# ratschlab/secedo

Hardware: AMD Instinct MI355X
Metric: cell-pair x locus updates/sec (similarity matrix) (higher is better)
Workload: dtype int64

## Files before the change

### secedo_amd/csrc/pack_device.hip

```cpp
#include "pack_device.hpp"

#include <hip/hip_runtime.h>
#include <hipcub/hipcub.hpp>

#include <algorithm>
#include <chrono>
#include <cstdio>
#include <cstdlib>
#include <cstring>

namespace secedo {

DeviceArena::~DeviceArena() {
    if (p) (void)hipFree(p);
}

DevicePacked::~DevicePacked() {
    if (side) (void)hipStreamDestroy(side);
    if (ev_fork) (void)hipEventDestroy(ev_fork);
    if (ev_join) (void)hipEventDestroy(ev_join);
    if (ev_offsets) (void)hipEventDestroy(ev_offsets);
    if (ev_flush) (void)hipEventDestroy(ev_flush);
    if (mailbox) (void)hipHostFree(mailbox);
}
// ... 861 lines not shown
            if (split[t] != cut) {
                split[t] = cut;
                sc->split_changed = 1;
            }
            l_prev = l_t;
        }
    }
}

__device__ __forceinline__ unsigned long long bin_key(uint32_t blk, uint32_t l, uint32_t cib, uint32_t lbits) {
    return ((((unsigned long long)blk << lbits) | l) << kCibBits) | cib;
}

__global__ void k_keys2(Raw in, const uint32_t *sval, const unsigned long long *incl,
                        const uint32_t *read_locus, const uint32_t *run_rank, const uint32_t *read_off,
                        uint32_t num_cells, uint32_t B,
                        uint32_t lbits, unsigned long long *key2, uint32_t *val2, uint32_t *t_read,
                        uint32_t *krank, uint8_t *kflags, unsigned long long *entry_kc, const uint32_t *entry_map,
                        uint32_t *blk_cnt_add, uint32_t L, Scalars *sc) {
    const uint32_t n = in.n_entries;
    for (uint32_t s = blockIdx.x * TPB + threadIdx.x; s < n; s += gridDim.x * TPB) {
        const unsigned long long cur = incl[s], prev = s ? incl[s - 1] : 0ull;
        const uint32_t e_out = entry_map ? entry_map[sval[s]] : sval[s];
        if (incl_kept(cur) == incl_kept(prev)) {
            if (entry_kc) entry_kc[e_out] = kNoEntry;
            continue;
        }
        const uint32_t k = incl_kept(prev);
        const uint32_t group = in.id_base(sval[s]) >> 2;
        uint32_t cell = 0;
        if (group >= in.n_groups) {
            sc->error = 1;
        } else {
            cell = in.g2p[group];
            if (cell >= num_cells) {
                sc->error = 2;
                cell = 0;
            }
        }
        const uint32_t blk = cell / B, cib = cell - blk * B;
        if (key2) {
            key2[k] = bin_key(blk, read_locus[k], cib, lbits);
            val2[k] = k;
        }
        const uint32_t r = incl_reads(cur) - 1;
        t_read[k] = r;
        krank[k] = run_rank[r];
        kflags[k] = (uint8_t)((in.id_base(sval[s]) & 3u) | (read_off[r + 1] - read_off[r] > 1u ? 4u : 0u));
        if (entry_kc) entry_kc[e_out] = ((unsigned long long)((blk << kCibBits) | cib) << 32) | k;
        if (blk_cnt_add) atomicAdd(&blk_cnt_add[(size_t)blk * (L + 1) + read_locus[k]], 1u);
    }
}

__device__ __forceinline__ uint32_t tile_locus(const uint32_t *s_off, uint32_t lo, uint32_t hi, uint32_t e) {
    while (hi - lo > 1u) {
        const uint32_t mid = (lo + hi) >> 1;
        if (s_off[mid] <= e) lo = mid; else hi = mid;
    }
    return lo;
}

__global__ __launch_bounds__(TPB) void k_bin_hist(Raw in, uint32_t nb, uint32_t TL, unsigned long long *__restrict__ entry_kc,
                                                 const uint32_t *__restrict__ m_idx, uint32_t num_cells,
                                                 uint32_t B_log2, uint32_t *__restrict__ blk_cnt, Scalars *sc,
                                                 uint32_t g2p_lds) {
    extern __shared__ uint32_t lds_hist[];
    __shared__ uint32_t s_off[65];
    static_assert(TPB >= 65, "one thread per offset");
    const uint32_t L = in.n_loci, TLP = TL + 1u, TL_log2 = 31u - (uint32_t)__clz((int)TL);
    const uint32_t n_tiles = (L + TL - 1u) / TL;
    constexpr int U = 4;
    uint16_t *s_g2p = reinterpret_cast<uint16_t *>(lds_hist + nb * TLP);
    if (g2p_lds) {
        for (uint32_t i = threadIdx.x; i < in.n_groups; i += TPB) s_g2p[i] = (uint16_t)min(in.g2p[i], 0xFFFFu);
    }
    for (uint32_t tile = blockIdx.x; tile < n_tiles; tile += gridDim.x) {
        const uint32_t l0 = tile * TL, n_l = min(TL, L - l0);
        for (uint32_t i = threadIdx.x; i < nb * TLP; i += TPB) lds_hist[i] = 0;
        if (threadIdx.x <= n_l) s_off[threadIdx.x] = (uint32_t)in.locus_entry_off[l0 + threadIdx.x];
        __syncthreads();
        const uint32_t eb = s_off[0], ee = s_off[n_l];
        for (uint32_t base = eb + threadIdx.x; base < ee; base += TPB * U) {
            uint32_t slot[U];
            constexpr uint32_t kNone = 0xFFFFFFFFu;
            if (m_idx) {
                uint32_t m0[U], m1[U], ib[U], cell[U];
#pragma unroll
                for (int u = 0; u < U; ++u) {
                    const uint32_t e = base + (uint32_t)u * TPB;
                    const bool in_tile = e < ee;
                    m0[u] = in_tile ? m_idx[e] : 0u;
                    m1[u] = in_tile ? m_idx[e + 1] : 1u;
                    ib[u] = in_tile ? in.id_base(e) : 0u;
                }
#pragma unroll
                for (int u = 0; u < U; ++u) {
                    const uint32_t group = ib[u] >> 2;
                    cell[u] = 0;
                    if (m1[u] == m0[u]) {
                        if (group >= in.n_groups) sc->error = 1;
                        else cell[u] = g2p_lds ? (uint32_t)s_g2p[group] : in.g2p[group];
                    }
                }
#pragma unroll
                for (int u = 0; u < U; ++u) {
                    slot[u] = kNone;
                    if (m1[u] != m0[u]) continue;
                    const uint32_t e = base + (uint32_t)u * TPB;
                    uint32_t c = cell[u];
                    if (c >= num_cells) {
                        sc->error = 2;
                        c = 0;
                    }
                    const uint32_t blk = c >> B_log2, cib = c - (blk << B_log2);
                    entry_kc[e] = ((unsigned long long)(((ib[u] & 3u) << kSingleBaseShift) | (blk << kCibBits) | cib) << 32)
                            | kSingle;
                    slot[u] = blk;
                }
            } else {
#pragma unroll
                for (int u = 0; u < U; ++u) {
                    const uint32_t e = base + (uint32_t)u * TPB;
                    const unsigned long long kc = e < ee ? entry_kc[e] : (unsigned long long)kNoEntry;
                    slot[u] = (uint32_t)kc != kNoEntry ? (uint32_t)(kc >> 32) >> kCibBits : kNone;
                }
            }
#pragma unroll
            for (int u = 0; u < U; ++u) {
                if (slot[u] == kNone) continue;
                const uint32_t j = tile_locus(s_off, 0u, n_l, base + (uint32_t)u * TPB);
                atomicAdd(&lds_hist[slot[u] * TLP + j], 1u);
            }
        }
        __syncthreads();
        for (uint32_t i = threadIdx.x; i < nb * TL; i += TPB) {
            const uint32_t b = i >> TL_log2, j = i & (TL - 1u);
            if (j < n_l) {
                blk_cnt[(size_t)b * (L + 1) + l0 + j] = lds_hist[b * TLP + j];
                if (l0 + j == L - 1) blk_cnt[(size_t)b * (L + 1) + L] = 0;
            }
        }
        __syncthreads();
    }
}

__global__ __launch_bounds__(TPB) void k_bin_place(Raw in, uint32_t nb, uint32_t TL,
                                                  const unsigned long long *__restrict__ entry_kc,
                                                  const uint32_t *__restrict__ blk_off, uint32_t B_log2, uint32_t bm_words,
                                                  const uint32_t *tail_begin,
                                                  unsigned long long *__restrict__ grouped, uint8_t *dupflag) {
    extern __shared__ uint32_t lds_hist[];
    __shared__ uint32_t s_off[65];
    __shared__ uint32_t s_tail[64];
    constexpr uint32_t NW = TPB / 64;
    constexpr int D = 4;
    const uint32_t lane = threadIdx.x & 63u, wv = threadIdx.x >> 6, L = in.n_loci, TLP = TL + 1u;
    const uint32_t TL_log2 = 31u - (uint32_t)__clz((int)TL);
    uint32_t *bm = lds_hist + nb * TLP + wv * bm_words;
    for (uint32_t i = lane; i < bm_words; i += 64u) bm[i] = 0;
    const uint32_t n_tiles = (L + TL - 1u) / TL;
    for (uint32_t tile = blockIdx.x; tile < n_tiles; tile += gridDim.x) {
        const uint32_t l0 = tile * TL, n_l = min(TL, L - l0);
        for (uint32_t i = threadIdx.x; i < nb * TL; i += TPB) {
            const uint32_t b = i >> TL_log2, j = i & (TL - 1u);
            if (j < n_l) lds_hist[b * TLP + j] = blk_off[(size_t)b * (L + 1) + l0 + j];
        }
        if (threadIdx.x <= n_l) s_off[threadIdx.x] = (uint32_t)in.locus_entry_off[l0 + threadIdx.x];
        if (threadIdx.x < n_l)
            s_tail[threadIdx.x] = tail_begin
                    ? tail_begin[last_le<uint32_t>(in.chr_locus_off, in.n_chr + 1, l0 + threadIdx.x)] : 0u;
        __syncthreads();
        const uint32_t per_wave = (n_l + NW - 1u) / NW;
        const uint32_t ja = min(n_l, wv * per_wave), jb = min(n_l, ja + per_wave);
        const uint32_t E0 = s_off[ja], E1 = s_off[jb];
        uint32_t cur = ja;
        bool twice = bm_words == 0u;
        auto close_locus = [&]() {
            const bool any_twice = __ballot(twice) != 0ull;
            if (lane == 0u) dupflag[l0 + cur] = any_twice ? 1 : 0;
            if (bm_words) {
                __builtin_amdgcn_fence(__ATOMIC_RELEASE, "wavefront");
                __builtin_amdgcn_wave_barrier();
                for (uint32_t i = lane; i < bm_words; i += 64u) bm[i] = 0;
                __builtin_amdgcn_fence(__ATOMIC_RELEASE, "wavefront");
                __builtin_amdgcn_wave_barrier();
            }
            twice = bm_words == 0u;
            ++cur;
        };
        auto chunk = [&](unsigned long long kc, uint32_t base) {
            const uint32_t e = base + lane;
            const bool valid = e < E1;
            const uint32_t j = valid ? tile_locus(s_off, cur, jb, e) : 0xFFFFFFFFu;
            const uint32_t chunk_end = min(E1, base + 64u);
            while (true) {
                if (valid && j == cur) {
                    uint32_t k = (uint32_t)kc;
                    if (k != kNoEntry) {
                        uint32_t cc = (uint32_t)(kc >> 32);
                        if (k & kSingle) {
                            k = kSingle | (e >= s_tail[cur] ? kSingleTail : 0u) | (cc >> kSingleBaseShift);
                            cc &= (1u << kSingleBaseShift) - 1u;
                        }
                        if (bm_words) {
                            const uint32_t cell = ((cc >> kCibBits) << B_log2) + (cc & ((1u << kCibBits) - 1u));
                            const uint32_t bit = 1u << (cell & 31u);
                            twice |= (atomicOr(&bm[cell >> 5], bit) & bit) != 0u;
                        }
                        const uint32_t pos = atomicAdd(&lds_hist[(cc >> kCibBits) * TLP + cur], 1u);
                        grouped[pos] = ((unsigned long long)((cc & ((1u << kCibBits) - 1u)) | ((l0 + cur) << kCibBits)) << 32) | k;
                    }
                }
                if (s_off[cur + 1] > chunk_end) break;
                close_locus();
                if (cur >= jb) break;
            }
        };
        unsigned long long ring[D];
#pragma unroll
        for (int d = 0; d < D; ++d) {
            const uint32_t e = E0 + (uint32_t)d * 64u + lane;
            ring[d] = e < E1 ? entry_kc[e] : (unsigned long long)kNoEntry;
        }
        for (uint32_t base = E0; base < E1; base += 64u * D) {
#pragma unroll
            for (int d = 0; d < D; ++d) {
                const uint32_t b = base + (uint32_t)d * 64u;
                if (b >= E1) break;
                const unsigned long long kc = ring[d];
                const uint32_t nxt = b + 64u * D + lane;
                ring[d] = nxt < E1 ? entry_kc[nxt] : (unsigned long long)kNoEntry;
                chunk(kc, b);
            }
        }
        while (cur < jb) close_locus();
        __syncthreads();
    }
}

__global__ __launch_bounds__(TPB) void k_group_counts(const unsigned long long *skey2, uint32_t n, uint32_t B,
                                                     uint32_t L, uint32_t lbits, uint32_t *blk_cnt,
                                                     unsigned long long *per_cell_sq) {
    constexpr uint32_t SLOTS = 512;
    __shared__ unsigned long long sq[SLOTS];
    __shared__ uint32_t first_cell;
    const uint32_t per_block = (n + gridDim.x - 1) / gridDim.x;
    const uint32_t d0 = blockIdx.x * per_block, d1 = min(n, d0 + per_block);
    for (uint32_t i = threadIdx.x; i < SLOTS; i += TPB) sq[i] = 0;
    if (threadIdx.x == 0 && d0 < n) {
        const unsigned long long key = skey2[d0];
        first_cell = (uint32_t)(key >> (kCibBits + lbits)) * B;
    }
    __syncthreads();
    for (uint32_t d = d0 + threadIdx.x; d < d1; d += TPB) {
        const unsigned long long key = skey2[d];
        const unsigned long long grp = key >> kCibBits;
        const uint32_t blk = (uint32_t)(grp >> lbits), l = (uint32_t)grp & ((1u << lbits) - 1u);
        if (d == 0 || skey2[d - 1] >> kCibBits != grp) {
            uint32_t len = 1;
            for (uint32_t t = d + 1; t < n && skey2[t] >> kCibBits == grp; ++t) ++len;
            blk_cnt[(size_t)blk * (L + 1) + l] = len;
        }
        if (d == 0 || skey2[d - 1] != key) {
            unsigned long long cnt = 1;
            for (uint32_t t = d + 1; t < n && skey2[t] == key; ++t) ++cnt;
            const uint32_t cell = blk * B + ((uint32_t)key & ((1u << kCibBits) - 1u));
            const uint32_t rel = cell - first_cell;
            if (rel < SLOTS) atomicAdd(&sq[rel], cnt * cnt);
            else atomicAdd(&per_cell_sq[cell], cnt * cnt);
        }
    }
    __syncthreads();
    if (d0 < n) {
        for (uint32_t i = threadIdx.x; i < SLOTS; i += TPB) {
            if (sq[i]) atomicAdd(&per_cell_sq[first_cell + i], sq[i]);
        }
    }
}

struct CapChoice {
    uint32_t entries_plain, loci_plain;
    uint32_t entries_counts, loci_counts;
    unsigned long long count_limit;
    uint32_t allow_counts;
    __device__ __forceinline__ bool counts(const Scalars *sc) const {
        return allow_counts && sc->pair_bound < count_limit;
    }
};

__global__ __launch_bounds__(TPB) void k_ranges_segment(const uint32_t *blk_off, uint32_t nb, uint32_t L,
// ... 124 lines not shown
        const uint32_t k = sval2[d];
        const uint32_t cib = (uint32_t)key & ((1u << kCibBits) - 1u);
        const unsigned long long grp = key >> kCibBits;
        const uint32_t blk = (uint32_t)(grp >> lbits), l = (uint32_t)grp & ((1u << lbits) - 1u);
        const uint32_t cell = blk * B + cib;
        const uint32_t fl = kflags[k];
        const uint32_t base = fl & 3u;
        const bool multi = (fl & 4u) != 0u;
        const uint32_t chr = locus_chr[l];
        const bool tail = krank[k] - rbeg[chr] >= flushed[chr];
        uint32_t r = 0, lo = k, hi = k + 1;
        if (multi) {
            r = t_read[k];
            lo = read_off[r];
            hi = read_off[r + 1];
        }
        uint32_t meta = cell | (base << kMetaBaseShift) | (tail ? kMetaTail : 0u);
        uint32_t masks = 0, bases = 0;
        bool wide = false;
        for (uint32_t j = k; j-- > lo;) {
            const uint32_t dist = l - read_locus[j];
            if (dist > kNarrowWindow) wide = true;
            if (dist > kWindow) {
                meta |= kMetaPrevOvf;
                break;
            }
            masks |= 1u << (dist - 1);
        }
        for (uint32_t j = k + 1; j < hi; ++j) {
            const uint32_t dist = read_locus[j] - l;
            if (dist > kNarrowWindow) wide = true;
            if (dist > kWindow) {
                meta |= kMetaNextOvf;
                break;
            }
            masks |= 1u << (16 + dist - 1);
            bases |= (uint32_t)(read_base[j] & 1u) << (dist - 1);
            bases |= (uint32_t)((read_base[j] >> 1) & 1u) << (16 + dist - 1);
        }
        if (multi || tail) {
            entry[d] = make_uint4(meta, masks, bases, l);
            entry_read[d] = r;
        }
        entry32[d] = cib | (base << kC_BaseShift) | (tail ? kC_Tail : 0u) | (multi ? kC_Multi : 0u)
                | (wide ? kC_Wide : 0u) | ((locus_rel[l] & 0xFFFFu) << 16);
        if (mask32)
            mask32[d] = (masks & 0xFFu) | (((masks >> 16) & 0xFFu) << 8) | ((bases & 0xFFu) << 16)
                    | (((bases >> 16) & 0xFFu) << 24);
        n_wide += wide ? 1u : 0u;
    }
    if (n_wide) atomicAdd(&sc->n_wide, n_wide);
}

constexpr uint32_t kRecMulti = 1u << 30, kRecWide = 1u << 31;
__global__ void k_m_records(Raw in, uint32_t n_kept_m, const uint32_t *t_read, const uint32_t *read_off,
                            const uint32_t *read_locus, const uint8_t *read_base, const uint32_t *krank,
                            const uint8_t *kflags, const uint32_t *rbeg, const uint32_t *flushed, uint4 *m_rec,
                            Scalars *sc) {
    __shared__ uint32_t s_chr[1025];
    const bool chr_lds = in.n_chr <= 1024u;
    if (chr_lds)
        for (uint32_t i = threadIdx.x; i <= in.n_chr; i += TPB) s_chr[i] = in.chr_locus_off[i];
    __syncthreads();
    uint32_t n_wide = 0;
    for (uint32_t k = blockIdx.x * TPB + threadIdx.x; k < n_kept_m; k += gridDim.x * TPB) {
        const uint32_t fl = kflags[k], l = read_locus[k];
        const bool multi = (fl & 4u) != 0u;
        const uint32_t chr = chr_lds ? last_le<uint32_t>(s_chr, in.n_chr + 1, l)
                                     : last_le<uint32_t>(in.chr_locus_off, in.n_chr + 1, l);
        const bool tail = krank[k] - rbeg[chr] >= flushed[chr];
        uint32_t r = 0, lo = k, hi = k + 1;
        if (multi) {
            r = t_read[k];
            lo = read_off[r];
            hi = read_off[r + 1];
        }
        uint32_t meta = ((fl & 3u) << kMetaBaseShift) | (tail ? kMetaTail : 0u) | (multi ? kRecMulti : 0u);
        uint32_t masks = 0, bases = 0;
        for (uint32_t j = k; j-- > lo;) {
            const uint32_t dist = l - read_locus[j];
            if (dist > kNarrowWindow) meta |= kRecWide;
            if (dist > kWindow) {
                meta |= kMetaPrevOvf;
                break;
            }
            masks |= 1u << (dist - 1);
        }
        for (uint32_t j = k + 1; j < hi; ++j) {
            const uint32_t dist = read_locus[j] - l;
            if (dist > kNarrowWindow) meta |= kRecWide;
            if (dist > kWindow) {
                meta |= kMetaNextOvf;
                break;
            }
            masks |= 1u << (16 + dist - 1);
            bases |= (uint32_t)(read_base[j] & 1u) << (dist - 1);
            bases |= (uint32_t)((read_base[j] >> 1) & 1u) << (16 + dist - 1);
        }
        m_rec[k] = make_uint4(meta, masks, bases, r);
        n_wide += (meta & kRecWide) ? 1u : 0u;
    }
    if (n_wide) atomicAdd(&sc->n_wide, n_wide);
}

struct RecordTables {
    const uint4 *m_rec;
    const uint32_t *locus_rel;
    uint4 *entry;
    uint32_t *entry32, *mask32, *entry_read;
};

__device__ __forceinline__ void emit_record(const RecordTables &t, uint32_t d, uint32_t k, uint4 rec, uint32_t cib,
                                            uint32_t cell, uint32_t l, uint32_t lrel) {
    uint32_t base, meta, masks = 0, bases = 0, r = 0;
    bool multi = false, wide = false, tail;
    if (k & kSingle) {
        base = k & 3u;
        tail = (k & kSingleTail) != 0u;
        meta = cell | (base << kMetaBaseShift) | (tail ? kMetaTail : 0u);
    } else {
        base = (rec.x >> kMetaBaseShift) & 3u;
        tail = (rec.x & kMetaTail) != 0u;
        multi = (rec.x & kRecMulti) != 0u;
        wide = (rec.x & kRecWide) != 0u;
        meta = cell | (rec.x & ~(kRecMulti | kRecWide));
        masks = rec.y;
        bases = rec.z;
        r = rec.w;
    }
    if (multi || tail) {
        t.entry[d] = make_uint4(meta, masks, bases, l);
        t.entry_read[d] = r;
    }
    t.entry32[d] = cib | (base << kC_BaseShift) | (tail ? kC_Tail : 0u) | (multi ? kC_Multi : 0u)
            | (wide ? kC_Wide : 0u) | (lrel << 16);
    if (t.mask32)
        t.mask32[d] = (masks & 0xFFu) | (((masks >> 16) & 0xFFu) << 8) | ((bases & 0xFFu) << 16)
                | (((bases >> 16) & 0xFFu) << 24);
}

constexpr int TPB_REC = 512;
__global__ __launch_bounds__(TPB_REC) void k_entry_records(const unsigned long long *grouped, const uint32_t *blk_off,
                                                          uint32_t n, uint32_t nb, uint32_t L, uint32_t B,
                                                          uint32_t lbits, RecordTables t,
                                                          unsigned long long *per_cell_sq, Scalars *sc) {
    constexpr uint32_t SLOTS = 512;
    __shared__ unsigned long long sq[SLOTS];
    __shared__ uint32_t blk_start[1025];
    __shared__ uint32_t first_cell;
    const uint32_t per_block = (n + gridDim.x - 1) / gridDim.x;
    const uint32_t d0 = blockIdx.x * per_block, d1 = min(n, d0 + per_block);
    for (uint32_t i = threadIdx.x; i < SLOTS; i += TPB_REC) sq[i] = 0;
    for (uint32_t i = threadIdx.x; i <= nb; i += TPB_REC) blk_start[i] = i < nb ? blk_off[(size_t)i * (L + 1)] : n;
    __syncthreads();
    auto block_of = [&](uint32_t p) {
        uint32_t lo = 0, hi = nb;
        while (hi - lo > 1) {
            const uint32_t mid = (lo + hi) >> 1;
            if (blk_start[mid] <= p) lo = mid; else hi = mid;
        }
        return lo;
    };
    if (threadIdx.x == 0 && d0 < n) first_cell = block_of(d0) * B;
    __syncthreads();
    const uint32_t lmask = (1u << lbits) - 1u;
    constexpr int U = 4;
    for (uint32_t base = d0; base < d1; base += TPB_REC * U) {
        unsigned long long mine[U];
        uint32_t blk[U], linfo[U], same[U];
        uint4 rec[U];
#pragma unroll
        for (int u = 0; u < U; ++u) {
            const uint32_t p = base + (uint32_t)u * TPB_REC + threadIdx.x;
            mine[u] = p < d1 ? grouped[p] : (unsigned long long)kSingle;
        }
#pragma unroll
        for (int u = 0; u < U; ++u) {
            const uint32_t p = base + (uint32_t)u * TPB_REC + threadIdx.x;
            const uint32_t l = (uint32_t)(mine[u] >> (32 + kCibBits)) & lmask;
            blk[u] = p < d1 ? block_of(p) : 0u;
            linfo[u] = t.locus_rel[l];
            rec[u] = make_uint4(0u, 0u, 0u, 0u);
            if (((uint32_t)mine[u] & kSingle) == 0u) rec[u] = t.m_rec[(uint32_t)mine[u]];
        }
#pragma unroll
        for (int u = 0; u < U; ++u) {
            const uint32_t p = base + (uint32_t)u * TPB_REC + threadIdx.x;
            same[u] = 1;
            if (p < d1 && (linfo[u] & kLocusDup)) {
                const uint32_t l = (uint32_t)(mine[u] >> (32 + kCibBits)) & lmask;
                const uint32_t cib = (uint32_t)(mine[u] >> 32) & ((1u << kCibBits) - 1u);
                const size_t g = (size_t)blk[u] * (L + 1) + l;
                const uint32_t gb = blk_off[g], ge = blk_off[g + 1];
// ... 25 lines not shown
            if (sq[i]) atomicAdd(&per_cell_sq[first_cell + i], sq[i]);
}

__global__ __launch_bounds__(TPB) void k_pair_bound(const unsigned long long *per_cell_sq, uint32_t n_cells_padded,
                                                   CapChoice caps, uint32_t assumed_counts, Scalars *sc) {
    __shared__ unsigned long long s_best[TPB / 64];
    unsigned long long best = 0;
    for (uint32_t i = threadIdx.x; i < n_cells_padded; i += TPB) best = max(best, per_cell_sq[i]);
    for (int off = 32; off > 0; off >>= 1) best = max(best, (unsigned long long)__shfl_down(best, off));
    if ((threadIdx.x & 63) == 0) s_best[threadIdx.x >> 6] = best;
    __syncthreads();
    if (threadIdx.x == 0) {
        for (int w = 1; w < TPB / 64; ++w) best = max(best, s_best[w]);
        sc->pair_bound = max(sc->pair_bound, best);
        sc->caps_wrong = (assumed_counts && !caps.counts(sc)) ? 1u : 0u;
    }
}

__global__ __launch_bounds__(TPB) void k_fix_locus_rel(const uint32_t *blk_off, uint32_t nb, uint32_t L,
                                                      const uint32_t *locus_rel, uint32_t *entry32) {
    const uint32_t n_groups = nb * (L + 1);
    for (uint32_t g = blockIdx.x * TPB + threadIdx.x; g < n_groups; g += gridDim.x * TPB) {
        const uint32_t l = g % (L + 1);
        if (l == L) continue;
        const uint32_t b = blk_off[g], e = blk_off[g + 1];
        if (b == e) continue;
        const uint32_t lrel = (locus_rel[l] & 0xFFFFu) << 16;
        for (uint32_t d = b; d < e; ++d) entry32[d] = (entry32[d] & 0xFFFFu) | lrel;
    }
}

int bits_for(unsigned long long max_value) {
    int b = 1;
    while (b < 64 && (max_value >> b) != 0) ++b;
    return b;
}

#define HIP_OK(expr)                                                                      \
    do {                                                                                  \
        hipError_t e__ = (expr);                                                          \
        if (e__ != hipSuccess) return std::string(#expr) + ": " + hipGetErrorString(e__); \
    } while (0)

std::string pack_attempt(const DeviceFlatPileup &in, uint32_t num_cells, uint32_t mfl, uint32_t num_threads,
                         uint32_t block_cells, StageGeometry (*geometry)(uint32_t), bool allow_count_tile,
                         bool force_radix, bool no_assumptions, hipStream_t stream, DevicePacked *out,
                         bool *need_host, int *retry) {
    *retry = kNoRetry;
    const uint32_t E = static_cast<uint32_t>(in.n_entries);
    const uint32_t L = in.n_loci, C = in.n_chr;
    DevicePacked &pk = *out;
    const size_t n_off_max = (size_t)((num_cells + 63) / 64) * ((size_t)L + 1);
    enum { KEY_A, KEY_B, VAL_A, VAL_B, ELOC, WORK_A, WORK_B, RUNS, CUB, TMP, MISC, BIN, ENTRY_KC,
           M_IDX, M_ENTRY, RID_M, IDB_M, ELOC_M, DENSE_M, MARK_M, ARANK_M, DUPF, SEGS };
    auto &S = pk.scratch;
    const size_t id_space_cap = std::min<size_t>((size_t)kIdSpaceFactor * E + 1024, (size_t)1 << 30);

    Raw raw{in.chr_locus_off, C, in.locus_pos, in.locus_entry_off, in.read_ids, in.id_base16,
            in.id_base32, in.group_id_to_pos, in.n_groups, L, E};

    HIP_OK(S[MISC].ensure(sizeof(Scalars) + sizeof(uint32_t) * ((size_t)7 * C + 4 + (size_t)4 * L) + 64));
    Scalars *sc = S[MISC].as<Scalars>();
    uint32_t *id_max = reinterpret_cast<uint32_t *>(sc + 1);
    uint32_t *id_negmin = id_max + C;
    uint32_t *id_base = id_negmin + C;
    uint32_t *rbeg = id_base + C + 1;
    uint32_t *flushed = rbeg + C + 1;
    uint32_t *cnt = flushed + C;
    uint32_t *locus_chr = cnt + L, *locus_rel = locus_chr + L;
    uint32_t *flush_loci = locus_rel + L, *flush_count = flush_loci + L;
    uint32_t *tail_begin = flush_count + C;
    HIP_OK(S[KEY_A].ensure(std::max<size_t>((size_t)E * 8, ((size_t)2 * E + 4 + n_off_max + 1) * 4)));
    HIP_OK(S[KEY_B].ensure((size_t)E * 8));
    HIP_OK(S[VAL_A].ensure(std::max<size_t>(E, 64) * 4));
    HIP_OK(S[VAL_B].ensure((size_t)E * 4));
    HIP_OK(S[ELOC].ensure((size_t)E * 4 + 16));
    HIP_OK(S[WORK_A].ensure(((size_t)E + 1) * 4));
    HIP_OK(S[WORK_B].ensure(((size_t)2 * E + 2) * 4));
    HIP_OK(S[RUNS].ensure(((size_t)3 * E + 8) * 4));
    HIP_OK(S[ENTRY_KC].ensure((size_t)E * 8));
    uint32_t *sloc = S[ENTRY_KC].as<uint32_t>();
    HIP_OK(S[TMP].ensure((size_t)E * 4 + 64));
    HIP_OK(S[BIN].ensure((size_t)E * 24 + ((size_t)num_cells + 130) * 8 + 64));
    unsigned long long *key_a = S[KEY_A].as<unsigned long long>(), *key_b = S[KEY_B].as<unsigned long long>();
    uint32_t *val_a = S[VAL_A].as<uint32_t>(), *val_b = S[VAL_B].as<uint32_t>();
    uint32_t *eloc = S[ELOC].as<uint32_t>();
    {
        size_t need = 0, most = 0;
        HIP_OK(hipcub::DeviceRadixSort::SortPairs(nullptr, need, key_a, key_b, val_a, val_b, (int)E, 0, 64, stream));
        most = std::max(most, need);
        {
            hipcub::CountingInputIterator<uint32_t> positions(0u);
            hipcub::TransformInputIterator<unsigned long long, HeadKeepOp, hipcub::CountingInputIterator<uint32_t>>
                    flags(positions, HeadKeepOp{key_b, val_a, val_a});
            HIP_OK(hipcub::DeviceScan::InclusiveSum(nullptr, need, flags, key_a, (int)E, stream));
            most = std::max(most, need);
        }
        HIP_OK(hipcub::DeviceScan::ExclusiveSum(nullptr, need, val_a, val_b, (int)E + 1, stream));
        most = std::max(most, need);
        HIP_OK(hipcub::DeviceScan::ExclusiveSum(nullptr, need, val_a, val_b,
                                                (int)std::max<size_t>(n_off_max, id_space_cap + 2), stream));
        most = std::max(most, need);
        HIP_OK(S[CUB].ensure(most + 1024));
    }
    void *cub_tmp = S[CUB].p;
    size_t cub_cap = 0;
    HIP_OK(hipMemsetAsync(sc, 0, sizeof(Scalars) + sizeof(uint32_t) * ((size_t)3 * C + 1), stream));
// ... 272 lines not shown
    pk.stage_masks = n_kept && (double)pk.multi_entries > geo.masks_threshold * (double)n_kept;

    uint32_t *t_read = S[TMP].as<uint32_t>();
    unsigned long long *key2_a = S[BIN].as<unsigned long long>();
    unsigned long long *key2_b = key2_a + nk;
    uint4 *m_rec = S[BIN].as<uint4>();
    unsigned long long *per_cell_sq = key2_b + nk;
    uint32_t *val2_a = reinterpret_cast<uint32_t *>(per_cell_sq + (size_t)nb * B + 1);
    uint32_t *val2_b = val2_a + nk;
    const size_t n_off = (size_t)nb * ((size_t)L + 1);
    uint32_t *blk_off = pk.blk_off.as<uint32_t>();
    uint32_t *blk_cnt = S[KEY_A].as<uint32_t>() + 2 * ((size_t)E + 1);
    unsigned long long *entry_kc = force_radix ? nullptr : S[ENTRY_KC].as<unsigned long long>();
    HIP_OK(S[DUPF].ensure((size_t)L + 16));
    uint8_t *dupflag = S[DUPF].as<uint8_t>();
    CapChoice caps;
    caps.entries_plain = pk.stage_masks ? geo.cap_entries_masks : geo.cap_entries_plain;
    caps.loci_plain = pk.stage_masks ? geo.cap_loci_masks : geo.cap_loci_plain;
    caps.entries_counts = geo.cap_entries_counts;
    caps.loci_counts = geo.cap_loci_counts;
    caps.count_limit = kCountTileLimit;
    caps.allow_counts = (allow_count_tile && !pk.stage_masks) ? 1u : 0u;
    if (caps.allow_counts && n_kept && L) {
        const double density = (double)n_kept / ((double)num_cells / B) / (double)L;
        const double per_segment = density * caps.loci_counts / caps.entries_counts;
        if (per_segment > 1.0) {
            const double greedy = std::ceil((double)L / caps.loci_counts) * std::ceil(per_segment);
            const uint32_t one = std::max(64u, (uint32_t)(0.93 * caps.entries_counts / density));
            if (one < caps.loci_counts && std::ceil((double)L / one) * 1.05 < greedy) caps.loci_counts = one;
        }
    }
    const uint32_t lo_loci = caps.allow_counts ? std::min(caps.loci_plain, caps.loci_counts) : caps.loci_plain;
    const uint32_t hi_loci = caps.allow_counts ? std::max(caps.loci_plain, caps.loci_counts) : caps.loci_plain;
    const uint32_t n_seg = (L + lo_loci - 1) / lo_loci;
    const size_t variant_stride = (size_t)n_seg * hi_loci + n_seg + 2;
    HIP_OK(S[SEGS].ensure(2 * variant_stride * 4));
    uint32_t *seg_count = S[SEGS].as<uint32_t>();
    uint32_t *seg_ends = seg_count + n_seg;
    auto cut_ranges_on_side = [&]() -> std::string {
        HIP_OK(hipEventRecord(pk.ev_offsets, stream));
        HIP_OK(hipStreamWaitEvent(pk.side, pk.ev_offsets, 0));
        hipLaunchKernelGGL(k_ranges_segment, dim3(n_seg, caps.allow_counts ? 2u : 1u), dim3(TPB), 0, pk.side, blk_off, nb,
                           L, caps, seg_ends, seg_count, variant_stride);
        HIP_OK(hipEventRecord(pk.ev_join, pk.side));
        return std::string();
    };
    if (force_radix) HIP_OK(hipMemsetAsync(blk_cnt, 0, (n_off + 1) * 4, stream));
    HIP_OK(hipMemsetAsync(per_cell_sq, 0, ((size_t)nb * B + 1) * 8, stream));
    uint32_t *krank = work_a;
    uint8_t *kflags = S[VAL_A].as<uint8_t>();
    uint32_t TL = 0, locus_grid = 0;
    size_t lds = 0;
    if (!force_radix) bin_tiles(nb, &TL, &locus_grid, &lds);
    const bool hist_first = split_singles && !force_radix;
    if (hist_first) {
        static const bool g2p_allowed = [] { const char *e = std::getenv("SECEDO_PACK_G2P_LDS"); return !(e && std::atoi(e) == 0); }();
        const size_t g2p_bytes = ((size_t)in.n_groups * 2 + 15) / 16 * 16;
        const bool g2p_lds = g2p_allowed && num_cells <= 0xFFFFu && lds + g2p_bytes <= 49152;
        hipLaunchKernelGGL(k_bin_hist, dim3(g2p_lds ? std::min<uint32_t>(locus_grid, 1024) : locus_grid), dim3(TPB),
                           lds + (g2p_lds ? g2p_bytes : 0), stream, raw, nb, TL, entry_kc, m_idx, num_cells, B_log2, blk_cnt,
                           sc, g2p_lds ? 1u : 0u);
    }
    if (n_m)
        hipLaunchKernelGGL(k_keys2, dim3(blocks_for(n_m)), dim3(TPB), 0, stream, sub, sval, incl, read_locus, run_rank,
                           read_off, num_cells, B, lbits, force_radix ? key2_a : nullptr, force_radix ? val2_a : nullptr,
                           t_read, krank, kflags, entry_kc, split_singles ? m_entry : nullptr,
                           hist_first ? blk_cnt : nullptr, L, sc);
    trace.mark("k_keys2 launched");
    const uint32_t slice_grid = std::min<uint32_t>(2048, (n_kept + 4095) / 4096);
    if (force_radix) {
        if (n_kept) {
            cub_cap = S[CUB].bytes;
            HIP_OK(hipcub::DeviceRadixSort::SortPairs(cub_tmp, cub_cap, key2_a, key2_b, val2_a, val2_b, (int)n_kept,
                                                       0, (int)(kCibBits + lbits) + bits_for(nb - 1), stream));
            hipLaunchKernelGGL(k_group_counts, dim3(slice_grid), dim3(TPB), 0, stream, key2_b, n_kept, B, L, lbits,
                               blk_cnt, per_cell_sq);
        }
        cub_cap = S[CUB].bytes;
        HIP_OK(hipcub::DeviceScan::ExclusiveSum(cub_tmp, cub_cap, blk_cnt, blk_off, (int)n_off, stream));
        const std::string err = cut_ranges_on_side();
        if (!err.empty()) return err;
    } else {
        if (!hist_first)
            hipLaunchKernelGGL(k_bin_hist, dim3(locus_grid), dim3(TPB), lds, stream, raw, nb, TL, entry_kc, nullptr, num_cells,
                               B_log2, blk_cnt, sc, 0u);
        trace.mark("k_bin_hist launched");
        const bool records_first = kept_m && (uint64_t)kept_m * 4u > (uint64_t)n_kept;
        if (records_first) {
            HIP_OK(hipEventRecord(pk.ev_offsets, stream));
            HIP_OK(hipStreamWaitEvent(pk.side, pk.ev_offsets, 0));
            hipLaunchKernelGGL(k_m_records, dim3(blocks_for(kept_m)), dim3(TPB), 0, pk.side, raw, kept_m, t_read, read_off,
                               read_locus, read_base, krank, kflags, rbeg, flushed, m_rec, sc);
            HIP_OK(hipEventRecord(pk.ev_join, pk.side));
        }
        cub_cap = S[CUB].bytes;
        HIP_OK(hipcub::DeviceScan::ExclusiveSum(cub_tmp, cub_cap, blk_cnt, blk_off, (int)n_off, stream));
        trace.mark("offset scan launched");
        if (records_first) {
            hipLaunchKernelGGL(k_ranges_segment, dim3(n_seg, caps.allow_counts ? 2u : 1u), dim3(TPB), 0, stream, blk_off, nb,
                               L, caps, seg_ends, seg_count, variant_stride);
        } else {
            const std::string err = cut_ranges_on_side();
            if (!err.empty()) return err;
            if (kept_m) {
                hipLaunchKernelGGL(k_m_records, dim3(blocks_for(kept_m)), dim3(TPB), 0, pk.side, raw, kept_m, t_read,
                                   read_off, read_locus, read_base, krank, kflags, rbeg, flushed, m_rec, sc);
                HIP_OK(hipEventRecord(pk.ev_join, pk.side));
            }
        }
        if (n_kept) {
            unsigned long long *grouped = key_b;
            HIP_OK(hipStreamWaitEvent(stream, pk.ev_flush, 0));
            uint32_t bm_words = (nb * B + 31) / 32;
            if (lds + (size_t)(TPB / 64) * bm_words * 4 > 49152) bm_words = 0;
            hipLaunchKernelGGL(k_bin_place, dim3(locus_grid), dim3(TPB), lds + (size_t)(TPB / 64) * bm_words * 4, stream,
                               raw, nb, TL, entry_kc, blk_off, B_log2, bm_words, split_singles ? tail_begin : nullptr,
                               grouped, dupflag);
        }
    }
    HIP_OK(hipStreamWaitEvent(stream, pk.ev_join, 0));
    side_join.joined = true;
    if (force_radix) {
        hipLaunchKernelGGL(k_ranges_compact, dim3(1), dim3(TPB), 0, stream, seg_ends, seg_count, variant_stride, n_seg,
                           caps, pk.range_off.as<uint32_t>(), per_cell_sq, n_kept ? nb * B : 0u, -1, sc);
        if (n_kept) {
            hipLaunchKernelGGL(k_locus_info, dim3(blocks_for(L)), dim3(TPB), 0, stream, raw, pk.range_off.as<uint32_t>(),
                               sc, nullptr, locus_chr, locus_rel);
            hipLaunchKernelGGL(k_records, dim3(blocks_for(n_kept)), dim3(TPB), 0, stream, raw, key2_b, val2_b, n_kept,
                               t_read, read_off, read_locus, read_base, krank, kflags, rbeg, flushed, locus_chr,
                               locus_rel, B, lbits, pk.entry.as<uint4>(), pk.entry32.as<uint32_t>(),
                               pk.stage_masks ? pk.mask32.as<uint32_t>() : nullptr, pk.entry_read.as<uint32_t>(), sc);
        }
    } else {
        const int assumed = caps.allow_counts ? 1 : 0;
        hipLaunchKernelGGL(k_ranges_compact, dim3(1), dim3(TPB), 0, stream, seg_ends, seg_count, variant_stride, n_seg,
                           caps, pk.range_off.as<uint32_t>(), per_cell_sq, 0u, assumed, sc);
        if (n_kept) {
            hipLaunchKernelGGL(k_locus_info, dim3(blocks_for(L)), dim3(TPB), 0, stream, raw, pk.range_off.as<uint32_t>(),
                               sc, dupflag, locus_chr, locus_rel);
            const RecordTables tables{m_rec, locus_rel, pk.entry.as<uint4>(), pk.entry32.as<uint32_t>(),
                                      pk.stage_masks ? pk.mask32.as<uint32_t>() : nullptr,
                                      pk.entry_read.as<uint32_t>()};
            const unsigned long long *grouped = key_b;
            hipLaunchKernelGGL(k_entry_records, dim3(std::min<uint32_t>(1u << 16, (n_kept + 4095) / 4096)), dim3(TPB_REC),
                               0, stream, grouped, blk_off, n_kept, nb, L, B, lbits, tables, per_cell_sq, sc);
        }
        hipLaunchKernelGGL(k_pair_bound, dim3(1), dim3(TPB), 0, stream, per_cell_sq, n_kept ? nb * B : 0u, caps,
                           (uint32_t)assumed, sc);
    }
    trace.mark("records launched");
    HIP_OK(read_scalars(pk, stream, sc, nullptr, &hsc, nullptr));
    trace.mark("read-back 3 arrived");
    if (!force_radix && hsc.caps_wrong && !hsc.regroup && hsc.error == 0) {
        hipLaunchKernelGGL(k_ranges_compact, dim3(1), dim3(TPB), 0, stream, seg_ends, seg_count, variant_stride, n_seg,
                           caps, pk.range_off.as<uint32_t>(), per_cell_sq, 0u, 0, sc);
        if (n_kept) {
            hipLaunchKernelGGL(k_locus_info, dim3(blocks_for(L)), dim3(TPB), 0, stream, raw, pk.range_off.as<uint32_t>(),
                               sc, nullptr, locus_chr, locus_rel);
            hipLaunchKernelGGL(k_fix_locus_rel, dim3(blocks_for(n_off)), dim3(TPB), 0, stream, blk_off, nb, L, locus_rel,
                               pk.entry32.as<uint32_t>());
        }
        HIP_OK(read_scalars(pk, stream, sc, nullptr, &hsc, nullptr));
    }
    if (hsc.error == 1) return "group id outside group_id_to_pos";
    if (hsc.error == 2) return "group_id_to_pos maps outside the matrix";
    if (hsc.regroup) {
        *retry = kRetryRadix;
        return std::string();
    }
    pk.pair_bound = hsc.pair_bound;
    pk.cell_sq = per_cell_sq;
    pk.cell_sq_n = n_kept ? nb * B : 0u;
    pk.cell_sq_host.clear();
    pk.count_tile = caps.allow_counts && pk.pair_bound < kCountTileLimit;
    pk.cap_entries = pk.count_tile ? caps.entries_counts : caps.entries_plain;
    pk.cap_loci = pk.count_tile ? caps.loci_counts : caps.loci_plain;
    pk.num_ranges = hsc.num_ranges;
    pk.n_wide = hsc.n_wide;
    HIP_OK(hipGetLastError());
    return std::string();
}

}

std::string pack_pileup_device(const DeviceFlatPileup &in, uint32_t num_cells, uint32_t mfl,
                               uint32_t num_threads, uint32_t block_cells,
                               StageGeometry (*geometry)(uint32_t), bool allow_count_tile,
                               hipStream_t stream, DevicePacked *out, bool *need_host) {
    *need_host = false;
    if ((in.id_base16 != nullptr) == (in.id_base32 != nullptr))
// ... 65 lines not shown
```

Measured before the change: 757.3 billion.

## Fuse record emission and per-cell square counts into bin placement kernel

Adds a templated fused path of k_bin_place that writes final entry records directly, instead of first writing an intermediate grouped array that k_entry_records later re-reads. The fused path also accumulates per-cell square counts in LDS, handling duplicate cell hits through a per-wave deferred list that scans earlier entries. Per-block LDS rows are then reduced by a small k_sq_rows kernel. This removes one kernel and a full pass over global memory, at the cost of more LDS use, possibly a smaller tile or grid, extra scans for duplicates, and added ordering complexity with the side stream.

```diff
diff --git a/secedo_amd/csrc/pack_device.hip b/secedo_amd/csrc/pack_device.hip
--- a/secedo_amd/csrc/pack_device.hip
+++ b/secedo_amd/csrc/pack_device.hip
@@ -937,6 +937,44 @@
     }
 }
 
+constexpr uint32_t kRecMulti = 1u << 30, kRecWide = 1u << 31;
+
+struct RecordTables {
+    const uint4 *m_rec;
+    const uint32_t *locus_rel;
+    uint4 *entry;
+    uint32_t *entry32, *mask32, *entry_read;
+};
+
+__device__ __forceinline__ void emit_record(const RecordTables &t, uint32_t d, uint32_t k, uint4 rec, uint32_t cib,
+                                            uint32_t cell, uint32_t l, uint32_t lrel) {
+    uint32_t base, meta, masks = 0, bases = 0, r = 0;
+    bool multi = false, wide = false, tail;
+    if (k & kSingle) {
+        base = k & 3u;
+        tail = (k & kSingleTail) != 0u;
+        meta = cell | (base << kMetaBaseShift) | (tail ? kMetaTail : 0u);
+    } else {
+        base = (rec.x >> kMetaBaseShift) & 3u;
+        tail = (rec.x & kMetaTail) != 0u;
+        multi = (rec.x & kRecMulti) != 0u;
+        wide = (rec.x & kRecWide) != 0u;
+        meta = cell | (rec.x & ~(kRecMulti | kRecWide));
+        masks = rec.y;
+        bases = rec.z;
+        r = rec.w;
+    }
+    if (multi || tail) {
+        t.entry[d] = make_uint4(meta, masks, bases, l);
+        t.entry_read[d] = r;
+    }
+    t.entry32[d] = cib | (base << kC_BaseShift) | (tail ? kC_Tail : 0u) | (multi ? kC_Multi : 0u)
+            | (wide ? kC_Wide : 0u) | (lrel << 16);
+    if (t.mask32)
+        t.mask32[d] = (masks & 0xFFu) | (((masks >> 16) & 0xFFu) << 8) | ((bases & 0xFFu) << 16)
+                | (((bases >> 16) & 0xFFu) << 24);
+}
+
 __device__ __forceinline__ uint32_t tile_locus(const uint32_t *s_off, uint32_t lo, uint32_t hi, uint32_t e) {
     while (hi - lo > 1u) {
         const uint32_t mid = (lo + hi) >> 1;
@@ -1029,20 +1067,66 @@
     }
 }
 
+constexpr uint32_t kAgainList = 64;
+template <bool FUSED>
 __global__ __launch_bounds__(TPB) void k_bin_place(Raw in, uint32_t nb, uint32_t TL,
                                                   const unsigned long long *__restrict__ entry_kc,
                                                   const uint32_t *__restrict__ blk_off, uint32_t B_log2, uint32_t bm_words,
                                                   const uint32_t *tail_begin,
-                                                  unsigned long long *__restrict__ grouped, uint8_t *dupflag) {
+                                                  unsigned long long *__restrict__ grouped, uint8_t *dupflag,
+                                                  RecordTables t, uint32_t sq_slots, uint32_t *sq_rows,
+                                                  unsigned long long *per_cell_sq, Scalars *sc) {
     extern __shared__ uint32_t lds_hist[];
     __shared__ uint32_t s_off[65];
     __shared__ uint32_t s_tail[64];
+    __shared__ uint32_t s_lrel[FUSED ? 64 : 1];
     constexpr uint32_t NW = TPB / 64;
     constexpr int D = 4;
     const uint32_t lane = threadIdx.x & 63u, wv = threadIdx.x >> 6, L = in.n_loci, TLP = TL + 1u;
     const uint32_t TL_log2 = 31u - (uint32_t)__clz((int)TL);
     uint32_t *bm = lds_hist + nb * TLP + wv * bm_words;
+    uint32_t *s_sq = lds_hist + nb * TLP + NW * bm_words;
+    uint2 *s_again = reinterpret_cast<uint2 *>(s_sq + sq_slots + (sq_slots & 1u)) + wv * kAgainList;
+    uint32_t n_again = 0;
+    auto add_sq = [&](uint32_t cell, uint32_t add) {
+        if (cell < sq_slots) {
+            const uint32_t old = atomicAdd(&s_sq[cell], add);
+            if ((unsigned long long)old + add > 0xFFFFFFFFull) atomicAdd(&per_cell_sq[cell], 1ull << 32);
+        } else {
+            atomicAdd(&per_cell_sq[cell], (unsigned long long)add);
+        }
+    };
+    auto drain = [&](uint32_t l0) {
+        if (n_again == 0u) return;
+        __atomic_signal_fence(__ATOMIC_SEQ_CST);
+        __builtin_amdgcn_s_waitcnt(0x0F70);
+        __atomic_signal_fence(__ATOMIC_SEQ_CST);
+        __builtin_amdgcn_wave_barrier();
+        for (uint32_t i = lane; i < n_again; i += 64u) {
+            const uint2 a = s_again[i];
+            const uint32_t pos = a.x, cell = a.y & 0xFFFFu, l = l0 + (a.y >> 16);
+            const uint32_t blk = cell >> B_log2, cib = cell - (blk << B_log2);
+            const size_t g = (size_t)blk * (L + 1) + l;
+            const uint32_t gb = blk_off[g], ge = blk_off[g + 1];
+            uint32_t add = 1;
+            if (ge - gb > kRankScanLimit) {
+                sc->regroup = 1;
+            } else {
+                uint32_t prev = 0;
+                for (uint32_t q = gb; q < pos; ++q)
+                    prev += (__hip_atomic_load(&t.entry32[q], __ATOMIC_RELAXED, __HIP_MEMORY_SCOPE_AGENT)
+                             & ((1u << kCibBits) - 1u)) == cib ? 1u : 0u;
+                add = 2u * prev + 1u;
+            }
+            add_sq(cell, add);
+        }
+        __builtin_amdgcn_fence(__ATOMIC_RELEASE, "wavefront");
+        __builtin_amdgcn_wave_barrier();
+        n_again = 0;
+    };
     for (uint32_t i = lane; i < bm_words; i += 64u) bm[i] = 0;
+    if (FUSED)
+        for (uint32_t i = threadIdx.x; i < sq_slots; i += TPB) s_sq[i] = 0;
     const uint32_t n_tiles = (L + TL - 1u) / TL;
     for (uint32_t tile = blockIdx.x; tile < n_tiles; tile += gridDim.x) {
         const uint32_t l0 = tile * TL, n_l = min(TL, L - l0);
@@ -1051,9 +1135,11 @@
             if (j < n_l) lds_hist[b * TLP + j] = blk_off[(size_t)b * (L + 1) + l0 + j];
         }
         if (threadIdx.x <= n_l) s_off[threadIdx.x] = (uint32_t)in.locus_entry_off[l0 + threadIdx.x];
-        if (threadIdx.x < n_l)
+        if (threadIdx.x < n_l) {
             s_tail[threadIdx.x] = tail_begin
                     ? tail_begin[last_le<uint32_t>(in.chr_locus_off, in.n_chr + 1, l0 + threadIdx.x)] : 0u;
+            if (FUSED) s_lrel[threadIdx.x] = t.locus_rel[l0 + threadIdx.x] & 0xFFFFu;
+        }
         __syncthreads();
         const uint32_t per_wave = (n_l + NW - 1u) / NW;
         const uint32_t ja = min(n_l, wv * per_wave), jb = min(n_l, ja + per_wave);
@@ -1062,7 +1148,7 @@
         bool twice = bm_words == 0u;
         auto close_locus = [&]() {
             const bool any_twice = __ballot(twice) != 0ull;
-            if (lane == 0u) dupflag[l0 + cur] = any_twice ? 1 : 0;
+            if (dupflag && lane == 0u) dupflag[l0 + cur] = any_twice ? 1 : 0;
             if (bm_words) {
                 __builtin_amdgcn_fence(__ATOMIC_RELEASE, "wavefront");
                 __builtin_amdgcn_wave_barrier();
@@ -1073,12 +1159,19 @@
             twice = bm_words == 0u;
             ++cur;
         };
-        auto chunk = [&](unsigned long long kc, uint32_t base) {
+        auto load_rec = [&](unsigned long long kc) {
+            const uint32_t k = (uint32_t)kc;
+            return (FUSED && k != kNoEntry && !(k & kSingle)) ? t.m_rec[k] : make_uint4(0u, 0u, 0u, 0u);
+        };
+        auto chunk = [&](unsigned long long kc, uint4 rec, uint32_t base) {
             const uint32_t e = base + lane;
             const bool valid = e < E1;
             const uint32_t j = valid ? tile_locus(s_off, cur, jb, e) : 0xFFFFFFFFu;
             const uint32_t chunk_end = min(E1, base + 64u);
             while (true) {
+                bool again = false;
+                bool placed = false;
+                uint32_t pos = 0, cell = 0, cib = 0, blk = 0;
                 if (valid && j == cur) {
                     uint32_t k = (uint32_t)kc;
                     if (k != kNoEntry) {
@@ -1087,13 +1180,34 @@
                             k = kSingle | (e >= s_tail[cur] ? kSingleTail : 0u) | (cc >> kSingleBaseShift);
                             cc &= (1u << kSingleBaseShift) - 1u;
                         }
+                        blk = cc >> kCibBits;
+                        cib = cc & ((1u << kCibBits) - 1u);
+                        cell = (blk << B_log2) + cib;
                         if (bm_words) {
-                            const uint32_t cell = ((cc >> kCibBits) << B_log2) + (cc & ((1u << kCibBits) - 1u));
                             const uint32_t bit = 1u << (cell & 31u);
-                            twice |= (atomicOr(&bm[cell >> 5], bit) & bit) != 0u;
+                            again = (atomicOr(&bm[cell >> 5], bit) & bit) != 0u;
+                            twice |= again;
                         }
-                        const uint32_t pos = atomicAdd(&lds_hist[(cc >> kCibBits) * TLP + cur], 1u);
-                        grouped[pos] = ((unsigned long long)((cc & ((1u << kCibBits) - 1u)) | ((l0 + cur) << kCibBits)) << 32) | k;
+                        pos = atomicAdd(&lds_hist[blk * TLP + cur], 1u);
+                        if (FUSED) {
+                            emit_record(t, pos, k, rec, cib, cell, l0 + cur, s_lrel[cur]);
+                            placed = true;
+                        } else {
+                            grouped[pos] = ((unsigned long long)(cib | ((l0 + cur) << kCibBits)) << 32) | k;
+                        }
+                    }
+                }
+                if (FUSED) {
+                    if (placed && !again) add_sq(cell, 1u);
+                    const unsigned long long ag = __ballot(again);
+                    if (ag) {
+                        const uint32_t cnt = (uint32_t)__popcll(ag);
+                        if (n_again + cnt > kAgainList) drain(l0);
+                        if (again) {
+                            const uint32_t slot = n_again + (uint32_t)__popcll(ag & ((1ull << lane) - 1ull));
+                            s_again[slot] = make_uint2(pos, (cur << 16) | cell);
+                        }
+                        n_again += cnt;
                     }
                 }
                 if (s_off[cur + 1] > chunk_end) break;
@@ -1102,25 +1216,45 @@
             }
         };
         unsigned long long ring[D];
+        uint4 ring_rec[D];
 #pragma unroll
         for (int d = 0; d < D; ++d) {
             const uint32_t e = E0 + (uint32_t)d * 64u + lane;
             ring[d] = e < E1 ? entry_kc[e] : (unsigned long long)kNoEntry;
         }
+        if (FUSED) ring_rec[0] = load_rec(ring[0]);
         for (uint32_t base = E0; base < E1; base += 64u * D) {
 #pragma unroll
             for (int d = 0; d < D; ++d) {
                 const uint32_t b = base + (uint32_t)d * 64u;
                 if (b >= E1) break;
                 const unsigned long long kc = ring[d];
+                const uint4 rec = FUSED ? ring_rec[d] : make_uint4(0u, 0u, 0u, 0u);
                 const uint32_t nxt = b + 64u * D + lane;
                 ring[d] = nxt < E1 ? entry_kc[nxt] : (unsigned long long)kNoEntry;
-                chunk(kc, b);
+                if (FUSED) ring_rec[(d + 1) % D] = load_rec(ring[(d + 1) % D]);
+                chunk(kc, rec, b);
             }
         }
         while (cur < jb) close_locus();
+        if (FUSED) {
+            __builtin_amdgcn_fence(__ATOMIC_RELEASE, "wavefront");
+            __builtin_amdgcn_wave_barrier();
+            drain(l0);
+        }
         __syncthreads();
     }
+    if (FUSED)
+        for (uint32_t i = threadIdx.x; i < sq_slots; i += TPB) sq_rows[(size_t)blockIdx.x * sq_slots + i] = s_sq[i];
+}
+
+__global__ __launch_bounds__(TPB) void k_sq_rows(const uint32_t *rows, uint32_t n_rows, uint32_t n_cells,
+                                                unsigned long long *per_cell_sq) {
+    const uint32_t c = blockIdx.x * TPB + threadIdx.x;
+    if (c >= n_cells) return;
+    unsigned long long sum = 0;
+    for (uint32_t r = blockIdx.y; r < n_rows; r += gridDim.y) sum += rows[(size_t)r * n_cells + c];
+    if (sum) atomicAdd(&per_cell_sq[c], sum);
 }
 
 __global__ __launch_bounds__(TPB) void k_group_counts(const unsigned long long *skey2, uint32_t n, uint32_t B,
@@ -1351,7 +1485,6 @@
     if (n_wide) atomicAdd(&sc->n_wide, n_wide);
 }
 
-constexpr uint32_t kRecMulti = 1u << 30, kRecWide = 1u << 31;
 __global__ void k_m_records(Raw in, uint32_t n_kept_m, const uint32_t *t_read, const uint32_t *read_off,
                             const uint32_t *read_locus, const uint8_t *read_base, const uint32_t *krank,
                             const uint8_t *kflags, const uint32_t *rbeg, const uint32_t *flushed, uint4 *m_rec,
@@ -1402,42 +1535,6 @@
     if (n_wide) atomicAdd(&sc->n_wide, n_wide);
 }
 
-struct RecordTables {
-    const uint4 *m_rec;
-    const uint32_t *locus_rel;
-    uint4 *entry;
-    uint32_t *entry32, *mask32, *entry_read;
-};
-
-__device__ __forceinline__ void emit_record(const RecordTables &t, uint32_t d, uint32_t k, uint4 rec, uint32_t cib,
-                                            uint32_t cell, uint32_t l, uint32_t lrel) {
-    uint32_t base, meta, masks = 0, bases = 0, r = 0;
-    bool multi = false, wide = false, tail;
-    if (k & kSingle) {
-        base = k & 3u;
-        tail = (k & kSingleTail) != 0u;
-        meta = cell | (base << kMetaBaseShift) | (tail ? kMetaTail : 0u);
-    } else {
-        base = (rec.x >> kMetaBaseShift) & 3u;
-        tail = (rec.x & kMetaTail) != 0u;
-        multi = (rec.x & kRecMulti) != 0u;
-        wide = (rec.x & kRecWide) != 0u;
-        meta = cell | (rec.x & ~(kRecMulti | kRecWide));
-        masks = rec.y;
-        bases = rec.z;
-        r = rec.w;
-    }
-    if (multi || tail) {
-        t.entry[d] = make_uint4(meta, masks, bases, l);
-        t.entry_read[d] = r;
-    }
-    t.entry32[d] = cib | (base << kC_BaseShift) | (tail ? kC_Tail : 0u) | (multi ? kC_Multi : 0u)
-            | (wide ? kC_Wide : 0u) | (lrel << 16);
-    if (t.mask32)
-        t.mask32[d] = (masks & 0xFFu) | (((masks >> 16) & 0xFFu) << 8) | ((bases & 0xFFu) << 16)
-                | (((bases >> 16) & 0xFFu) << 24);
-}
-
 constexpr int TPB_REC = 512;
 __global__ __launch_bounds__(TPB_REC) void k_entry_records(const unsigned long long *grouped, const uint32_t *blk_off,
                                                           uint32_t n, uint32_t nb, uint32_t L, uint32_t B,
@@ -1569,7 +1666,7 @@
     DevicePacked &pk = *out;
     const size_t n_off_max = (size_t)((num_cells + 63) / 64) * ((size_t)L + 1);
     enum { KEY_A, KEY_B, VAL_A, VAL_B, ELOC, WORK_A, WORK_B, RUNS, CUB, TMP, MISC, BIN, ENTRY_KC,
-           M_IDX, M_ENTRY, RID_M, IDB_M, ELOC_M, DENSE_M, MARK_M, ARANK_M, DUPF, SEGS };
+           M_IDX, M_ENTRY, RID_M, IDB_M, ELOC_M, DENSE_M, MARK_M, ARANK_M, DUPF, SEGS, SQ_ROWS };
     auto &S = pk.scratch;
     const size_t id_space_cap = std::min<size_t>((size_t)kIdSpaceFactor * E + 1024, (size_t)1 << 30);
 
@@ -1948,6 +2045,15 @@
     uint32_t TL = 0, locus_grid = 0;
     size_t lds = 0;
     if (!force_radix) bin_tiles(nb, &TL, &locus_grid, &lds);
+    static const bool fused_allowed = [] {
+        const char *e = std::getenv("SECEDO_PACK_FUSED_RECORDS");
+        return !(e && std::atoi(e) == 0);
+    }();
+    static const bool sq_lds_allowed = [] {
+        const char *e = std::getenv("SECEDO_PACK_SQ_LDS");
+        return !(e && std::atoi(e) == 0);
+    }();
+    bool fused = false;
     const bool hist_first = split_singles && !force_radix;
     if (hist_first) {
         static const bool g2p_allowed = [] { const char *e = std::getenv("SECEDO_PACK_G2P_LDS"); return !(e && std::atoi(e) == 0); }();
@@ -1982,7 +2088,24 @@
                                B_log2, blk_cnt, sc, 0u);
         trace.mark("k_bin_hist launched");
         const bool records_first = kept_m && (uint64_t)kept_m * 4u > (uint64_t)n_kept;
-        if (records_first) {
+        uint32_t bm_words = (nb * B + 31) / 32;
+        if (lds + (size_t)(TPB / 64) * bm_words * 4 > 49152) bm_words = 0;
+        fused = n_kept && bm_words && !records_first && fused_allowed;
+        constexpr size_t kPlaceLds = 54272 - 1024;
+        const uint32_t n_cells_b = nb * B;
+        auto place_lds = [&](uint32_t tl, uint32_t slots) {
+            return (size_t)nb * (tl + 1) * 4 + (size_t)(TPB / 64) * bm_words * 4 + ((size_t)slots + 1) * 4
+                    + (size_t)(TPB / 64) * kAgainList * 8;
+        };
+        uint32_t TLp = TL, sq_slots = sq_lds_allowed ? n_cells_b : 0u;
+        while (TLp > 16 && place_lds(TLp, sq_slots) > kPlaceLds) TLp >>= 1;
+        if (place_lds(TLp, sq_slots) > kPlaceLds) {
+            TLp = TL;
+            sq_slots = place_lds(TL, 0) < kPlaceLds
+                    ? (uint32_t)std::min<size_t>(sq_slots, (kPlaceLds - place_lds(TL, 0)) / 4) : 0u;
+        }
+        if (sq_lds_allowed && sq_slots < n_cells_b) fused = false;
+        if (records_first || (fused && kept_m)) {
             HIP_OK(hipEventRecord(pk.ev_offsets, stream));
             HIP_OK(hipStreamWaitEvent(pk.side, pk.ev_offsets, 0));
             hipLaunchKernelGGL(k_m_records, dim3(blocks_for(kept_m)), dim3(TPB), 0, pk.side, raw, kept_m, t_read, read_off,
@@ -1992,7 +2115,7 @@
         cub_cap = S[CUB].bytes;
         HIP_OK(hipcub::DeviceScan::ExclusiveSum(cub_tmp, cub_cap, blk_cnt, blk_off, (int)n_off, stream));
         trace.mark("offset scan launched");
-        if (records_first) {
+        if (records_first || fused) {
             hipLaunchKernelGGL(k_ranges_segment, dim3(n_seg, caps.allow_counts ? 2u : 1u), dim3(TPB), 0, stream, blk_off, nb,
                                L, caps, seg_ends, seg_count, variant_stride);
         } else {
@@ -2004,14 +2127,33 @@
                 HIP_OK(hipEventRecord(pk.ev_join, pk.side));
             }
         }
-        if (n_kept) {
+        if (fused) {
+            hipLaunchKernelGGL(k_ranges_compact, dim3(1), dim3(TPB), 0, stream, seg_ends, seg_count, variant_stride, n_seg,
+                               caps, pk.range_off.as<uint32_t>(), per_cell_sq, 0u, caps.allow_counts ? 1 : 0, sc);
+            hipLaunchKernelGGL(k_locus_info, dim3(blocks_for(L)), dim3(TPB), 0, stream, raw, pk.range_off.as<uint32_t>(),
+                               sc, nullptr, locus_chr, locus_rel);
+            HIP_OK(hipStreamWaitEvent(stream, pk.ev_join, 0));
+            const RecordTables tables{m_rec, locus_rel, pk.entry.as<uint4>(), pk.entry32.as<uint32_t>(),
+                                      pk.stage_masks ? pk.mask32.as<uint32_t>() : nullptr,
+                                      pk.entry_read.as<uint32_t>()};
+            const uint32_t place_grid = std::min<uint32_t>((L + TLp - 1) / TLp, sq_slots ? 1024u : 8192u);
+            uint32_t *sq_rows = nullptr;
+            if (sq_slots) {
+                HIP_OK(S[SQ_ROWS].ensure((size_t)place_grid * sq_slots * 4));
+                sq_rows = S[SQ_ROWS].as<uint32_t>();
+            }
+            hipLaunchKernelGGL(k_bin_place<true>, dim3(place_grid), dim3(TPB), place_lds(TLp, sq_slots), stream, raw, nb,
+                               TLp, entry_kc, blk_off, B_log2, bm_words, split_singles ? tail_begin : nullptr, nullptr,
+                               nullptr, tables, sq_slots, sq_rows, per_cell_sq, sc);
+            if (sq_slots)
+                hipLaunchKernelGGL(k_sq_rows, dim3((sq_slots + TPB - 1) / TPB, 32), dim3(TPB), 0, stream, sq_rows, place_grid,
+                                   sq_slots, per_cell_sq);
+        } else if (n_kept) {
             unsigned long long *grouped = key_b;
             HIP_OK(hipStreamWaitEvent(stream, pk.ev_flush, 0));
-            uint32_t bm_words = (nb * B + 31) / 32;
-            if (lds + (size_t)(TPB / 64) * bm_words * 4 > 49152) bm_words = 0;
-            hipLaunchKernelGGL(k_bin_place, dim3(locus_grid), dim3(TPB), lds + (size_t)(TPB / 64) * bm_words * 4, stream,
-                               raw, nb, TL, entry_kc, blk_off, B_log2, bm_words, split_singles ? tail_begin : nullptr,
-                               grouped, dupflag);
+            hipLaunchKernelGGL(k_bin_place<false>, dim3(locus_grid), dim3(TPB), lds + (size_t)(TPB / 64) * bm_words * 4,
+                               stream, raw, nb, TL, entry_kc, blk_off, B_log2, bm_words,
+                               split_singles ? tail_begin : nullptr, grouped, dupflag, RecordTables{}, 0u, nullptr, nullptr, sc);
         }
     }
     HIP_OK(hipStreamWaitEvent(stream, pk.ev_join, 0));
@@ -2029,9 +2171,10 @@
         }
     } else {
         const int assumed = caps.allow_counts ? 1 : 0;
-        hipLaunchKernelGGL(k_ranges_compact, dim3(1), dim3(TPB), 0, stream, seg_ends, seg_count, variant_stride, n_seg,
-                           caps, pk.range_off.as<uint32_t>(), per_cell_sq, 0u, assumed, sc);
-        if (n_kept) {
+        if (!fused)
+            hipLaunchKernelGGL(k_ranges_compact, dim3(1), dim3(TPB), 0, stream, seg_ends, seg_count, variant_stride, n_seg,
+                               caps, pk.range_off.as<uint32_t>(), per_cell_sq, 0u, assumed, sc);
+        if (n_kept && !fused) {
             hipLaunchKernelGGL(k_locus_info, dim3(blocks_for(L)), dim3(TPB), 0, stream, raw, pk.range_off.as<uint32_t>(),
                                sc, dupflag, locus_chr, locus_rel);
             const RecordTables tables{m_rec, locus_rel, pk.entry.as<uint4>(), pk.entry32.as<uint32_t>(),
```

Measured after the change: 764.1 billion, median of 6. No clear change (+0.9%).
